# ShinYwings/SingleHDR-tf2

Measured on AMD Instinct MI355X. Metric: HDR images/sec (512x512) end-to-end inference, deq+lin+hal, higher is better.
Workload: dtype f32

## Files before the change

include/shdr.h:

```cpp
#ifndef SHDR_H_
#define SHDR_H_

#include <stdint.h>

#ifdef __cplusplus
extern "C" {
#endif

void shdr_config_reload(void);

#define SHDR_OK          0
#define SHDR_E_SHAPE    (-1)
#define SHDR_E_ALIGN    (-2)
#define SHDR_E_ARCH     (-3)
#define SHDR_E_LAUNCH   (-4)
#define SHDR_E_NULL     (-5)

#define SHDR_ACT_NONE   0
#define SHDR_ACT_RELU   1
#define SHDR_ACT_LRELU  2
#define SHDR_ACT_TANH   3

#define SHDR_ALGO_AUTO    0
#define SHDR_ALGO_MFMA    1
// ... 59 lines not shown
int64_t shdr_conv2d_workspace_bytes_f32(const shdr_conv2d_desc* d, int has_residual);
int shdr_conv2d_fwd_prepared_f32(const shdr_conv2d_desc* d, const float* x1, const float* x2, const float* prepared,
                                 const float* bias, const float* scale, const float* shift, const float* residual, float* y,
                                 float* y_pool, void* workspace, void* stream);
int shdr_conv2d_fwd_prepared_ranged_f32(const shdr_conv2d_desc* d, const float* x1, const float* x2, const float* prepared,
                                        const float* bias, const float* scale, const float* shift, const float* residual, float* y,
                                        float* y_pool, void* workspace, const float* x1_range, const float* x2_range, float* y_range,
                                        void* stream);
int shdr_conv2d_projected_ok_f32(const shdr_conv2d_desc* d);
int shdr_conv2d_fwd_prepared_projected_f32(const shdr_conv2d_desc* d, const float* x1, const float* x2, const float* prepared,
                                           const float* bias, const float* scale, const float* shift, const float* proj, float* y_proj,
                                           float* y, float* y_pool, void* workspace, const float* x1_range, const float* x2_range,
                                           float* y_range, void* stream);

int shdr_conv2d_up2_lowres_ok_f32(const shdr_conv2d_desc* d);
int64_t shdr_conv2d_up2_lowres_filter_elems_f32(const shdr_conv2d_desc* d);
int shdr_conv2d_up2_lowres_prepare_filter_f32(const shdr_conv2d_desc* d, const float* w, float* prepared, void* stream);
int64_t shdr_conv2d_up2_lowres_workspace_bytes_f32(const shdr_conv2d_desc* d);
int shdr_conv2d_fwd_up2_lowres_f32(const shdr_conv2d_desc* d, const float* x, const float* prepared, const float* bias,
                                   const float* scale, const float* shift, float* y, void* workspace, const float* x_range,
                                   float* y_range, void* stream);

int shdr_conv2d_up2_fused_ok_f32(const shdr_conv2d_desc* d);
int64_t shdr_conv2d_up2_fused_filter_elems_f32(const shdr_conv2d_desc* d);
int shdr_conv2d_up2_fused_prepare_filter_f32(const shdr_conv2d_desc* d, const float* w, float* prepared, void* stream);
int shdr_conv2d_fwd_up2_fused_f32(const shdr_conv2d_desc* d, const float* x, const float* prepared, const float* bias,
                                  const float* scale, const float* shift, const float* proj, float* y_proj, float* y,
                                  const float* x_range, float* y_range, void* stream);

int shdr_conv2d_wgrad_f32(const shdr_conv2d_desc* d, const float* x, int which, const float* dz,
                          float* dw, void* stream);
int shdr_filter_transform_f32(const float* w, float* wt, int KH, int KW, int Cin, int Cout,
                              int c_begin, int c_count, float scale, void* stream);
int64_t shdr_conv2d_dgrad_workspace_bytes_f32(const shdr_conv2d_desc* d, int which);
int shdr_conv2d_dgrad_f32(const shdr_conv2d_desc* d, int which, const float* dz, const float* w, float* dx, void* workspace,
                          void* stream);
int shdr_conv2d_dgrad_tracks_range_f32(const shdr_conv2d_desc* d, int which);
int shdr_conv2d_dgrad_ranged_f32(const shdr_conv2d_desc* d, int which, const float* dz, const float* w, float* dx, void* workspace,
                                 const float* dz_range, float* dx_range, void* stream);
enum { SHDR_OP_CONV2D_FWD = 0, SHDR_OP_CONV2D_DGRAD = 1, SHDR_OP_CONV2D_WGRAD_WINOGRAD = 2, SHDR_OP_BATCHNORM = 3,
       SHDR_OP_ACT_BWD_BIAS = 4  };
#define SHDR_BN_MAX_BLOCKS 1024
int64_t shdr_workspace_bytes(int op, const shdr_conv2d_desc* d, int arg);
int shdr_bias_grad_f32(const float* dz, float* db, int64_t npix, int C, void* stream);

int shdr_soft_hist_fwd_f32(const float* x, float* y, int64_t npix, int C, int B, void* stream);
// ... 358 lines not shown
```

singlehdr-tf2_amd/_lib.py:

```python
import ctypes
import os

_HERE = os.path.dirname(os.path.abspath(__file__))
LIB_PATH = os.environ.get("SHDR_LIB") or os.path.join(_HERE, "libshdr.so")

c_int = ctypes.c_int
c_i64 = ctypes.c_int64
c_f32 = ctypes.c_float
c_ptr = ctypes.c_void_p


class ConvDesc(ctypes.Structure):
    _fields_ = [("N", ctypes.c_int32), ("H", ctypes.c_int32), ("W", ctypes.c_int32),
                ("C1", ctypes.c_int32), ("C2", ctypes.c_int32),
                ("Cout", ctypes.c_int32), ("KH", ctypes.c_int32), ("KW", ctypes.c_int32),
                ("stride", ctypes.c_int32), ("pad_t", ctypes.c_int32), ("pad_l", ctypes.c_int32),
                ("Ho", ctypes.c_int32), ("Wo", ctypes.c_int32),
                ("x2_scale", ctypes.c_float),
                ("act1", ctypes.c_int32), ("act2", ctypes.c_int32),
                ("res_cstride", ctypes.c_int32), ("y_cstride", ctypes.c_int32),
                ("algo", ctypes.c_int32), ("cout_valid", ctypes.c_int32),
                ("w_batch_stride", ctypes.c_int64),
                ("y_pix_stride", ctypes.c_int32), ("y_off_h", ctypes.c_int32), ("y_off_w", ctypes.c_int32),
                ("y_H", ctypes.c_int32), ("y_W", ctypes.c_int32),
# ... 63 lines not shown
    "shdr_conv2d_fwd_x3n_ranged_f32": (c_int, [ctypes.POINTER(ConvDesc)] + [c_ptr] * 13),
    "shdr_act_bwd_bias_f32": (c_int, [c_ptr, c_ptr, c_ptr, c_ptr, c_ptr, c_i64, c_int, c_int, c_ptr]),
    "shdr_winograd_filter_packed_f32": (c_int, [c_ptr, c_ptr, c_int, c_int, c_ptr]),
    "shdr_conv2d_wgrad_winograd_f32": (c_int, [c_ptr] * 4 + [c_int] * 7 + [c_f32, c_ptr]),
    "shdr_crc32c": (ctypes.c_uint32, [c_ptr, ctypes.c_uint64, ctypes.c_uint32]),
    "shdr_same_pad": (c_int, [c_int, c_int, c_int, ctypes.POINTER(c_int), ctypes.POINTER(c_int)]),
    "shdr_conv2d_fwd_f32": (c_int, [ctypes.POINTER(ConvDesc)] + [c_ptr] * 9),
    "shdr_conv2d_fwd_yrange_f32": (c_int, [ctypes.POINTER(ConvDesc)] + [c_ptr] * 10),
    "shdr_conv2d_plan_f32": (c_int, [ctypes.POINTER(ConvDesc), c_int]),
    "shdr_conv2d_prepared_filter_elems_f32": (c_i64, [ctypes.POINTER(ConvDesc), c_int]),
    "shdr_conv2d_filter_is_plain_f32": (c_int, [ctypes.POINTER(ConvDesc), c_int]),
    "shdr_conv2d_prepare_filter_f32": (c_int, [ctypes.POINTER(ConvDesc), c_int, c_ptr, c_ptr, c_ptr]),
    "shdr_conv2d_workspace_bytes_f32": (c_i64, [ctypes.POINTER(ConvDesc), c_int]),
    "shdr_conv2d_fwd_prepared_f32": (c_int, [ctypes.POINTER(ConvDesc)] + [c_ptr] * 11),
    "shdr_conv2d_fwd_prepared_ranged_f32": (c_int, [ctypes.POINTER(ConvDesc)] + [c_ptr] * 14),
    "shdr_conv2d_projected_ok_f32": (c_int, [ctypes.POINTER(ConvDesc)]),
    "shdr_conv2d_fwd_prepared_projected_f32": (c_int, [ctypes.POINTER(ConvDesc)] + [c_ptr] * 15),
    "shdr_conv2d_up2_lowres_ok_f32": (c_int, [ctypes.POINTER(ConvDesc)]),
    "shdr_conv2d_up2_lowres_filter_elems_f32": (c_i64, [ctypes.POINTER(ConvDesc)]),
    "shdr_conv2d_up2_lowres_prepare_filter_f32": (c_int, [ctypes.POINTER(ConvDesc), c_ptr, c_ptr, c_ptr]),
    "shdr_conv2d_up2_lowres_workspace_bytes_f32": (c_i64, [ctypes.POINTER(ConvDesc)]),
    "shdr_conv2d_fwd_up2_lowres_f32": (c_int, [ctypes.POINTER(ConvDesc)] + [c_ptr] * 10),
    "shdr_conv2d_up2_fused_ok_f32": (c_int, [ctypes.POINTER(ConvDesc)]),
    "shdr_conv2d_up2_fused_filter_elems_f32": (c_i64, [ctypes.POINTER(ConvDesc)]),
    "shdr_conv2d_up2_fused_prepare_filter_f32": (c_int, [ctypes.POINTER(ConvDesc), c_ptr, c_ptr, c_ptr]),
    "shdr_conv2d_fwd_up2_fused_f32": (c_int, [ctypes.POINTER(ConvDesc)] + [c_ptr] * 11),
    "shdr_conv2d_fwd_x3_projected_f32": (c_int, [ctypes.POINTER(ConvDesc)] + [c_ptr] * 14),
    "shdr_conv2d_fwd_x3_residual_f32": (c_int, [ctypes.POINTER(ConvDesc)] + [c_ptr] * 12),
    "shdr_conv2d_dgrad_workspace_bytes_f32": (c_i64, [ctypes.POINTER(ConvDesc), c_int]),
    "shdr_conv2d_dgrad_f32": (c_int, [ctypes.POINTER(ConvDesc), c_int, c_ptr, c_ptr, c_ptr, c_ptr, c_ptr]),
    "shdr_conv2d_dgrad_tracks_range_f32": (c_int, [ctypes.POINTER(ConvDesc), c_int]),
    "shdr_conv2d_dgrad_ranged_f32": (c_int, [ctypes.POINTER(ConvDesc), c_int, c_ptr, c_ptr, c_ptr, c_ptr, c_ptr, c_ptr, c_ptr]),
    "shdr_workspace_bytes": (c_i64, [c_int, ctypes.POINTER(ConvDesc), c_int]),
    "shdr_soft_hist_bwd_f32": (c_int, [c_ptr, c_ptr, c_ptr, c_i64, c_int, c_int, c_ptr]),
    "shdr_conv2d_wgrad_f32": (c_int, [ctypes.POINTER(ConvDesc), c_ptr, c_int, c_ptr, c_ptr, c_ptr]),
    "shdr_filter_transform_f32": (c_int, [c_ptr, c_ptr, c_int, c_int, c_int, c_int, c_int, c_int, c_f32, c_ptr]),
    "shdr_bias_grad_f32": (c_int, [c_ptr, c_ptr, c_i64, c_int, c_ptr]),
    "shdr_soft_hist_fwd_f32": (c_int, [c_ptr, c_ptr, c_i64, c_int, c_int, c_ptr]),
    "shdr_lin_frontend_fwd_f32": (c_int, [c_ptr, c_ptr, c_int, c_int, c_int, c_int, c_ptr]),
    "shdr_avgpool2_fwd_f32": (c_int, [c_ptr, c_ptr, c_int, c_int, c_int, c_int, c_ptr]),
    "shdr_maxpool2_fwd_f32": (c_int, [c_ptr, c_ptr, c_int, c_int, c_int, c_int, c_ptr]),
    "shdr_maxpool3s2_fwd_f32": (c_int, [c_ptr, c_ptr, c_int, c_int, c_int, c_int, c_ptr]),
    "shdr_resize2x_fwd_f32": (c_int, [c_ptr, c_ptr, c_int, c_int, c_int, c_int, c_ptr]),
    "shdr_gap_fwd_f32": (c_int, [c_ptr, c_ptr, c_int, c_int, c_int, c_ptr]),
    "shdr_invcrf_decode_fwd_f32": (c_int, [c_ptr] * 5 + [c_int, c_int, c_int, c_ptr]),
    "shdr_increase_fwd_f32": (c_int, [c_ptr, c_ptr, c_int, c_int, c_ptr]),
# ... 116 lines not shown
```

singlehdr-tf2_amd/_ops.py:

```python
import collections
import ctypes
import math

import numpy as np
import torch

try:
    from . import _lib
except ImportError:
    import _lib

AUTOGRAD = None


def _needs_grad(*tensors):
    return AUTOGRAD is not None and torch.is_grad_enabled() and any(
        isinstance(t, torch.Tensor) and t.requires_grad for t in tensors)


WINOGRAD = True


ACT_NONE, ACT_RELU, ACT_LRELU, ACT_TANH = 0, 1, 2, 3
ALGO_AUTO, ALGO_MFMA, ALGO_DIRECT, ALGO_MFMA_REG = 0, 1, 2, 3
# ... 165 lines not shown
            raise NotImplementedError("conv2d: the native-fp16 path takes no pad / out / w_batch_stride / algo")
        if _needs_grad(x, x2, w, bias, scale, shift, residual):
            if fused:
                raise NotImplementedError("conv2d: the native-fp16 path takes bias + act1 only on a gradient tape (training-mode layers)")
            return AUTOGRAD.conv2d_h(x, w, bias, stride, x2, x2_scale, act1, cout_valid)
        return conv2d_h(x, pack_filter_h(w, x.shape[3], 0 if x2 is None else x2.shape[3], x2_scale), bias, tuple(w.shape[:2]),
                        w.shape[3], stride=stride, x2=x2, act1=act1, cout_valid=cout_valid, scale=scale, shift=shift,
                        residual=residual, act2=act2)
    if algo == ALGO_AUTO:
        algo = _AUTO_ALGO[PRECISION]
    fused = scale is not None or shift is not None or residual is not None or act2 != ACT_NONE
    if _needs_grad(x, x2, w, bias, scale, shift, residual):
        if pad is not None or out_hw is not None or out is not None or w_batch_stride:
            raise NotImplementedError("conv2d: pad / out_hw / out / w_batch_stride are raw-kernel options (input-gradient and "
                                      "Winograd plumbing) and cannot be recorded on a gradient tape")
        y = AUTOGRAD.conv2d(x, w, bias, stride=stride, x2=x2, x2_scale=x2_scale, act1=act1, algo=algo, cout_valid=cout_valid)
        if not fused:
            return y
        return AUTOGRAD.affine_act(y, scale, shift, residual, act2)
    return _conv2d_raw(x, w, bias, stride, x2, x2_scale, act1, scale, shift, residual, act2, algo, out, cout_valid, pad, out_hw,
                       w_batch_stride, None)


def conv2d_up2(x, w, bias=None, act1=ACT_NONE, scale=None, shift=None, act2=ACT_NONE, proj=None, lowres=False):
    if lowres and proj is not None and not _is_h(x) and _AUTO_ALGO[PRECISION] == ALGO_AUTO and WINOGRAD and not EXACT_FP32 \
            and not _needs_grad(x, w, bias, scale, shift):
        yj = _conv2d_up2_fused(x, w, bias, act1, scale, shift, act2, proj)
        if yj is not None:
            return yj
    if lowres and proj is None and not _is_h(x) and _AUTO_ALGO[PRECISION] == ALGO_AUTO and WINOGRAD and not EXACT_FP32 \
            and not _needs_grad(x, w, bias, scale, shift):
        y = _conv2d_up2_lowres(x, w, bias, act1, scale, shift, act2)
        if y is not None:
            return y
    algo = _AUTO_ALGO[PRECISION]
    if _is_h(x) or algo != ALGO_AUTO or not WINOGRAD or _needs_grad(x, w, bias, scale, shift):
        if proj is not None:
            return None
        return conv2d(resize2x(x), w, bias, act1=act1, scale=scale, shift=shift, act2=act2)
    return _conv2d_raw(x, w, bias, 1, None, 1.0, act1, scale, shift, None, act2, algo, None, None, None, None, 0, None,
                       prologue=PROLOGUE_BILINEAR2X, proj=proj)


def _up2_layer(form, x, w, bias, act1, scale, shift, act2):
    lib = _lib.load()
    x, w_var = _d(x), w
    w = _d(w)
    if x.dim() != 4 or w.dim() != 4 or tuple(w.shape[:2]) != (3, 3) or w.shape[2] != x.shape[3]:
        return None
    n, h, wd, c1 = x.shape
    cout = w.shape[3]
    d = _lib.ConvDesc()
    d.N, d.H, d.W, d.C1, d.C2 = n, 2 * h, 2 * wd, c1, 0
    d.Cout, d.KH, d.KW, d.stride = cout, 3, 3, 1
    d.cout_valid, d.y_cstride = cout, cout
    d.pad_t, d.pad_l, d.Ho, d.Wo = 1, 1, 2 * h, 2 * wd
    d.x2_scale = 1.0
    d.act1, d.act2 = act1, act2
    d.algo = ALGO_AUTO
    d.prologue = PROLOGUE_BILINEAR2X
    if not int(getattr(lib, "shdr_conv2d_up2_%s_ok_f32" % form)(ctypes.byref(d))):
        return None
    _chk(x, "x")
    _chk(w, "w")
# ... 13 lines not shown
    return d, x, prepared


def _conv2d_up2_lowres(x, w, bias, act1, scale, shift, act2):
    layer = _up2_layer("lowres", x, w, bias, act1, scale, shift, act2)
    if layer is None:
        return None
    lib = _lib.load()
    x_in = x
    d, x, prepared = layer
    xr = _range_of(x_in)
    if xr is None:
        RANGE_MISSES[(tuple(x.shape), None, tuple(_d(w).shape))] += 1
    ws = torch.empty(int(lib.shdr_conv2d_up2_lowres_workspace_bytes_f32(ctypes.byref(d))), device=x.device, dtype=torch.uint8)
    out = torch.empty((d.N, d.H, d.W, d.Cout), device=x.device, dtype=torch.float32)
    yr = _new_slot(x.device)
    rc = lib.shdr_conv2d_fwd_up2_lowres_f32(ctypes.byref(d), _ptr(x), _ptr(prepared), _ptr(_d(bias)), _ptr(_d(scale)), _ptr(_d(shift)),
                                            _ptr(out), _ptr(ws), _ptr(xr), _ptr(yr), _stream())
    _lib.check(rc, "shdr_conv2d_fwd_up2_lowres_f32")
    return _set_range(out, yr)


def _conv2d_up2_fused(x, w, bias, act1, scale, shift, act2, proj=None, want_y=None):
    layer = _up2_layer("fused", x, w, bias, act1, scale, shift, act2)
    if layer is None:
        return None
    lib = _lib.load()
    x_in = x
    d, x, prepared = layer
    if proj is not None:
        proj = _chk(_d(proj), "proj")
        if tuple(proj.shape) != (3, d.Cout):
            raise ValueError("conv2d_up2: proj must be [3, %d]" % d.Cout)
    if want_y is None:
        want_y = proj is None
    xr = _range_of(x_in)
    if xr is None:
        RANGE_MISSES[(tuple(x.shape), None, tuple(_d(w).shape))] += 1
        xr = _new_slot(x.device)
        _lib.check(lib.shdr_absmax_f32(_ptr(x), x.numel(), _ptr(xr), _stream()), "shdr_absmax_f32")
    out = torch.empty((d.N, d.H, d.W, d.Cout), device=x.device, dtype=torch.float32) if want_y else None
    yj = torch.empty((d.N, d.H, d.W, 3), device=x.device, dtype=torch.float32) if proj is not None else None
    yr = _new_slot(x.device) if want_y else None
    rc = lib.shdr_conv2d_fwd_up2_fused_f32(ctypes.byref(d), _ptr(x), _ptr(prepared), _ptr(_d(bias)), _ptr(_d(scale)), _ptr(_d(shift)),
                                           _ptr(proj), _ptr(yj), _ptr(out), _ptr(xr), _ptr(yr), _stream())
    _lib.check(rc, "shdr_conv2d_fwd_up2_fused_f32")
# ... 1843 lines not shown
```

singlehdr-tf2_amd/csrc/up2_fused.hip:

```cpp
#include <hip/hip_fp16.h>
#include <stdlib.h>

#include <type_traits>

#include "shdr_internal.h"

namespace {

using f32x4 = __attribute__((ext_vector_type(4))) float;
using f16x8 = __attribute__((ext_vector_type(8))) _Float16;

inline hipStream_t S(void* s) { return reinterpret_cast<hipStream_t>(s); }

constexpr int UF_HEADER_FLOATS = 16;
constexpr int UF_IMG_HALVES = 64 * 32, UF_UNIT_HALVES = 2 * UF_IMG_HALVES;
constexpr int UF_R = 8;
constexpr int UF_COLS = 14;
constexpr int UF_MAX_CIN = 128;
constexpr int UF_STRIDE = UF_MAX_CIN + 8;
constexpr int UF_THREADS = 256;

struct UpFusedArgs {
  const float* x;
  const _Float16* wp;
  const float* hdr;
  const float* bias;
  const float* scale;
  const float* shift;
  const float* proj;
  float* y;
  float* yproj;
  const unsigned* xr;
  unsigned* yr;
  int N, h, w, C1, nty, ntx, act1, act2;
};

__device__ __forceinline__ void uf_range_scale(const unsigned* r, float& xs, float& ixs) {
  xs = 1.0f;
  ixs = 1.0f;
  const unsigned b = r ? *r : 0u;
  if (b != 0u && b < 0x7f800000u) {
    int ex;
    frexpf(__uint_as_float(b), &ex);
    int T = 11 - ex;
    T = T < -126 ? -126 : (T > 126 ? 126 : T);
    xs = ldexpf(1.0f, T);
    ixs = ldexpf(1.0f, -T);
  }
}
__device__ __forceinline__ void uf_split4(const f32x4 v, float xs, unsigned (&h)[2], unsigned (&l)[2]) {
  const float k2048 = 2048.0f;
#pragma unroll
  for (int p = 0; p < 2; ++p) {
    float t0, t1;
    asm("v_fma_mixlo_f16 %0, %1, %2, 0" : "=v"(h[p]) : "v"(v[2 * p]), "s"(xs));
    asm("v_fma_mixhi_f16 %0, %1, %2, 0" : "+v"(h[p]) : "v"(v[2 * p + 1]), "s"(xs));
    asm("v_fma_mix_f32 %0, %1, %2, -%3 op_sel_hi:[0,0,1]" : "=v"(t0) : "v"(v[2 * p]), "s"(xs), "v"(h[p]));
// ... 19 lines not shown
  f32x4 r;
#pragma unroll
  for (int e = 0; e < 4; ++e) r[e] = __builtin_fmaf(a[e], s[e], c[e]);
  return r;
}
__device__ __forceinline__ f32x4 from_left(f32x4 a) {
  f32x4 r;
#pragma unroll
  for (int e = 0; e < 4; ++e) r[e] = __int_as_float(__builtin_amdgcn_update_dpp(0, __float_as_int(a[e]), 0x111, 0xf, 0xf, true));
  return r;
}
__device__ __forceinline__ f32x4 from_right(f32x4 a) {
  f32x4 r;
#pragma unroll
  for (int e = 0; e < 4; ++e) r[e] = __int_as_float(__builtin_amdgcn_update_dpp(0, __float_as_int(a[e]), 0x101, 0xf, 0xf, true));
  return r;
}

__device__ __forceinline__ int uf_xcd_remap(int bid, int nwg) {
  const int q = nwg >> 3, r = nwg & 7, xcd = bid & 7, idx = bid >> 3;
  return (xcd < r ? xcd * (q + 1) : r * (q + 1) + (xcd - r) * q) + idx;
}

template <int R>
__global__ __launch_bounds__(UF_THREADS, 2) void up2_fused_kernel(const UpFusedArgs a) {
  constexpr int NPIX = 16 * R, IMG = NPIX * UF_STRIDE;
  constexpr int RO = R - 2;
  extern __shared__ __attribute__((aligned(16))) _Float16 fsm[];

  const int tid = threadIdx.x, lane = tid & 63;
  const int cw = __builtin_amdgcn_readfirstlane(tid >> 6);
  int L = uf_xcd_remap(blockIdx.x, gridDim.x);
  const int tx_ = L % a.ntx; L /= a.ntx;
  const int ty_ = L % a.nty;
  const int n = L / a.nty;
  const int m_start = ty_ * RO, j_start = tx_ * UF_COLS;
  const int nch = a.C1 >> 5;

  float xs, ixs;
  {
    const int f4n = a.C1 >> 2, total = NPIX * f4n;
    const float* xb = a.x + (size_t)n * a.h * a.w * a.C1;
    uf_range_scale(a.xr, xs, ixs);
#pragma unroll 1
    for (int id0 = tid; id0 < total; id0 += 4 * UF_THREADS) {
      f32x4 v[4];
      int dst[4];
#pragma unroll
      for (int k = 0; k < 4; ++k) {
        const int id = id0 + k * UF_THREADS;
        dst[k] = -1;
        if (id < total) {
          const int pp = id / f4n, f = id - pp * f4n;
          const int row = min(max(m_start - 1 + (pp >> 4), 0), a.h - 1), col = min(max(j_start - 1 + (pp & 15), 0), a.w - 1);
          v[k] = *reinterpret_cast<const f32x4*>(xb + ((size_t)row * a.w + col) * a.C1 + 4 * f);
          dst[k] = pp * UF_STRIDE + 4 * f;
        }
      }
#pragma unroll
      for (int k = 0; k < 4; ++k) {
        if (dst[k] >= 0) {
          unsigned h[2], l[2];
          uf_split4(v[k], xs, h, l);
          *reinterpret_cast<uint2*>(fsm + dst[k]) = make_uint2(h[0], h[1]);
          *reinterpret_cast<uint2*>(fsm + IMG + dst[k]) = make_uint2(l[0], l[1]);
        }
      }
    }
  }
  __syncthreads();

  const int p = lane & 15, fg = lane >> 4;
  const int j0 = j_start - 1 + p;
  const bool lane_ok = p >= 1 && p <= UF_COLS && j0 < a.w;
  const float wl0 = j0 >= 1 ? 0.75f : 0.0f, wl1 = j0 >= 1 ? 0.25f : 0.0f;
  const float wr0 = j0 + 1 < a.w ? 0.25f : 0.0f, wr1 = j0 + 1 < a.w ? 0.75f : 0.0f;
  const float inv_s = a.hdr[1] * ixs;
  const _Float16* wlane = a.wp + (16 * cw + p) * 32 + 8 * fg;
  const _Float16* xlane = fsm + p * UF_STRIDE + 8 * fg;

  f32x4 out[RO][2][2];

  auto pass = [&](auto tyc) __attribute__((always_inline)) {
    constexpr int TY = decltype(tyc)::value;
    f32x4 z[3][R];
#pragma unroll
    for (int t = 0; t < 3; ++t)
#pragma unroll
      for (int q = 0; q < R; ++q) z[t][q] = (f32x4){0.f, 0.f, 0.f, 0.f};
    const _Float16* wt = wlane + (size_t)(3 * TY) * nch * UF_UNIT_HALVES;
#pragma unroll 1
    for (int c = 0; c < nch; ++c) {
      f16x8 wh[3], wl[3], ws[3];
#pragma unroll
      for (int t = 0; t < 3; ++t) {
        const _Float16* g = wt + ((size_t)t * nch + c) * UF_UNIT_HALVES;
        wh[t] = *reinterpret_cast<const f16x8*>(g);
        wl[t] = *reinterpret_cast<const f16x8*>(g + UF_IMG_HALVES);
      }
#pragma unroll
      for (int t = 0; t < 3; ++t) ws[t] = wh[t] * (_Float16)(1.0f / 2048.0f);
      const _Float16* xc = xlane + 32 * c;
#pragma unroll
      for (int q = 0; q < R; ++q) {
        const f16x8 ph = *reinterpret_cast<const f16x8*>(xc + q * 16 * UF_STRIDE);
        const f16x8 pl = *reinterpret_cast<const f16x8*>(xc + IMG + q * 16 * UF_STRIDE);
#pragma unroll
        for (int t = 0; t < 3; ++t) z[t][q] = __builtin_amdgcn_mfma_f32_16x16x32_f16(wh[t], ph, z[t][q], 0, 0, 0);
#pragma unroll
        for (int t = 0; t < 3; ++t) z[t][q] = __builtin_amdgcn_mfma_f32_16x16x32_f16(ws[t], pl, z[t][q], 0, 0, 0);
#pragma unroll
        for (int t = 0; t < 3; ++t) z[t][q] = __builtin_amdgcn_mfma_f32_16x16x32_f16(wl[t], ph, z[t][q], 0, 0, 0);
      }
    }
#pragma unroll
    for (int q = 0; q < R; ++q) {
      asm volatile("" : "+v"(z[0][q]), "+v"(z[1][q]), "+v"(z[2][q]));
      f32x4 zz[3];
#pragma unroll
// ... 31 lines not shown
        } else if (TY == 1) {
          if (q >= 2) out[q - 2][1][s] = fma4(H[s], 0.25f, out[q - 2][1][s]);
          if (q + 1 <= RO) out[q][0][s] = fma4(H[s], 0.25f, out[q][0][s]);
          if (q >= 1 && q <= RO) {
            out[q - 1][0][s] = fma4(H[s], 0.75f, out[q - 1][0][s]);
            out[q - 1][1][s] = fma4(H[s], 0.75f, out[q - 1][1][s]);
          }
        } else {
          if (q >= 2) {
            out[q - 2][0][s] = fma4(H[s], 0.25f, out[q - 2][0][s]);
            out[q - 2][1][s] = fma4(H[s], mq < a.h ? 0.75f : 0.0f, out[q - 2][1][s]);
          }
          if (q >= 1 && q <= RO) {
            out[q - 1][0][s] = fma4(H[s], 0.75f, out[q - 1][0][s]);
            out[q - 1][1][s] = fma4(H[s], mq + 1 < a.h ? 0.25f : 0.0f, out[q - 1][1][s]);
          }
        }
      }
      if (q >= 1 && q <= RO) asm volatile("" : "+v"(out[q - 1][0][0]), "+v"(out[q - 1][0][1]), "+v"(out[q - 1][1][0]), "+v"(out[q - 1][1][1]));
      if (q + 1 <= RO) asm volatile("" : "+v"(out[q][0][0]), "+v"(out[q][0][1]), "+v"(out[q][1][0]), "+v"(out[q][1][1]));
      if (q >= 2) asm volatile("" : "+v"(out[q - 2][0][0]), "+v"(out[q - 2][0][1]), "+v"(out[q - 2][1][0]), "+v"(out[q - 2][1][1]));
    }
  };
  pass(std::integral_constant<int, 0>{});
  pass(std::integral_constant<int, 1>{});
  pass(std::integral_constant<int, 2>{});

  const int c = 16 * cw + 4 * fg;
  auto ld = [](const float* q) __attribute__((always_inline)) { return *reinterpret_cast<const f32x4*>(q); };
  const f32x4 bias_r = a.bias ? ld(a.bias + c) : (f32x4){0.f, 0.f, 0.f, 0.f};
  const f32x4 scale_r = a.scale ? ld(a.scale + c) : (f32x4){1.f, 1.f, 1.f, 1.f};
  const f32x4 shift_r = a.scale ? ld(a.shift + c) : (f32x4){0.f, 0.f, 0.f, 0.f};
  f32x4 pq[3];
#pragma unroll
  for (int j = 0; j < 3; ++j) pq[j] = a.proj ? ld(a.proj + j * 64 + c) : (f32x4){0.f, 0.f, 0.f, 0.f};
  if (a.proj) __syncthreads();
  float* part = reinterpret_cast<float*>(fsm);
  float ym = 0.0f;
#pragma unroll
  for (int qo = 0; qo < RO; ++qo) {
    const int m0 = m_start + qo;
    const bool row_ok = m0 < a.h;
#pragma unroll
    for (int r = 0; r < 2; ++r)
#pragma unroll
      for (int s = 0; s < 2; ++s) {
        f32x4 v = out[qo][r][s];
        v += bias_r;
        shdr::act_apply4<0>(v, a.act1);
        if (a.scale) v = fma4v(v, scale_r, shift_r);
        shdr::act_apply4<0>(v, a.act2);
        if (a.y && row_ok && lane_ok) {
          *reinterpret_cast<f32x4*>(a.y + (((size_t)n * 2 * a.h + 2 * m0 + r) * 2 * a.w + 2 * j0 + s) * 64 + c) = v;
          ym = fmaxf(fmaxf(fmaxf(fmaxf(ym, fabsf(v[0])), fabsf(v[1])), fabsf(v[2])), fabsf(v[3]));
        }
        if (a.proj) {
#pragma unroll
          for (int j = 0; j < 3; ++j) {
            float t = v[0] * pq[j][0] + v[1] * pq[j][1] + v[2] * pq[j][2] + v[3] * pq[j][3];
            t += __shfl_xor(t, 16, 64);
            t += __shfl_xor(t, 32, 64);
            if (fg == 0) part[(cw * RO * 64 + (qo * 2 + r) * 32 + 2 * p + s) * 3 + j] = t;
          }
        }
      }
  }
  if (a.proj) {
    __syncthreads();
    for (int slot = tid; slot < RO * 64; slot += UF_THREADS) {
      const int s = slot & 1, pp = (slot >> 1) & 15, r = (slot >> 5) & 1, qo = slot >> 6;
      const int m0 = m_start + qo, jj = j_start - 1 + pp;
      if (m0 < a.h && pp >= 1 && pp <= UF_COLS && jj < a.w) {
        float* o = a.yproj + (((size_t)n * 2 * a.h + 2 * m0 + r) * 2 * a.w + 2 * jj + s) * 3;
#pragma unroll
        for (int j = 0; j < 3; ++j)
          o[j] = ((part[slot * 3 + j] + part[(RO * 64 + slot) * 3 + j]) + part[(2 * RO * 64 + slot) * 3 + j]) + part[(3 * RO * 64 + slot) * 3 + j];
      }
    }
  }
  if (a.y && a.yr) shdr::range_out_block256(a.yr, ym);
}

constexpr int uf_lds_bytes(int R) { return 2 * 16 * R * UF_STRIDE * 2; }

bool uf_shape_ok(const shdr_conv2d_desc* d) {
  return d && d->N > 0 && d->H > 0 && d->W > 0 && d->H % 2 == 0 && d->W % 2 == 0 && d->KH == 3 && d->KW == 3 && d->stride == 1 && d->pad_t == 1 &&
         d->pad_l == 1 && d->Ho == d->H && d->Wo == d->W && d->C2 == 0 && d->C1 % 32 == 0 && d->C1 >= 64 && d->C1 <= UF_MAX_CIN && d->Cout == 64;
}

}

extern "C" int shdr_conv2d_up2_fused_ok_f32(const shdr_conv2d_desc* d) {
  if (!uf_shape_ok(d) || SHDR_ENV("SHDR_NO_UP2_FUSED") != nullptr || SHDR_ENV("SHDR_NO_UP2_LOWRES") != nullptr || SHDR_ENV("SHDR_NO_WINOGRAD") != nullptr ||
      SHDR_ENV("SHDR_NO_X3") != nullptr)
    return 0;
  if (d->algo != SHDR_ALGO_AUTO || d->prologue != SHDR_PROLOGUE_BILINEAR2X) return 0;
  if ((d->cout_valid != 0 && d->cout_valid != d->Cout) || d->w_batch_stride != 0 || d->y_pix_stride > 1 || (d->y_cstride != 0 && d->y_cstride != d->Cout)) return 0;
  if (d->act1 == SHDR_ACT_TANH || d->act2 == SHDR_ACT_TANH) return 0;
  const long nblk = (long)d->N * ((d->H / 2 + UF_R - 3) / (UF_R - 2)) * ((d->W / 2 + UF_COLS - 1) / UF_COLS);
  return nblk <= 0x7fffffffL ? 1 : 0;
}

extern "C" int64_t shdr_conv2d_up2_fused_filter_elems_f32(const shdr_conv2d_desc* d) {
  return uf_shape_ok(d) ? shdr_conv2d_up2_lowres_filter_elems_f32(d) : -1;
}
extern "C" int shdr_conv2d_up2_fused_prepare_filter_f32(const shdr_conv2d_desc* d, const float* w, float* prepared, void* stream) {
  SHDR_REQUIRE(uf_shape_ok(d), SHDR_E_SHAPE, "up2_fused_prepare_filter: need a 3x3 layer with one source, Cin 64 / 96 / 128, Cout 64, even H and W");
  return shdr_conv2d_up2_lowres_prepare_filter_f32(d, w, prepared, stream);
}

extern "C" int shdr_conv2d_fwd_up2_fused_f32(const shdr_conv2d_desc* d, const float* x, const float* prepared, const float* bias, const float* scale,
                                             const float* shift, const float* proj, float* y_proj, float* y, const float* x_range, float* y_range,
                                             void* stream) {
  SHDR_REQUIRE(d && x && prepared && x_range, SHDR_E_NULL, "conv2d_up2_fused: null desc / x / prepared filter / x_range");
  SHDR_REQUIRE(y || y_proj, SHDR_E_NULL, "conv2d_up2_fused: neither y nor y_proj");
  SHDR_REQUIRE((proj == nullptr) == (y_proj == nullptr), SHDR_E_NULL, "conv2d_up2_fused: proj and y_proj come together");
  SHDR_REQUIRE(shdr_conv2d_up2_fused_ok_f32(d), SHDR_E_SHAPE, "conv2d_up2_fused: layer not taken (shdr_conv2d_up2_fused_ok_f32)");
  SHDR_REQUIRE((scale == nullptr) == (shift == nullptr), SHDR_E_NULL, "conv2d_up2_fused: scale and shift come together");
  SHDR_REQUIRE(shdr::aligned16(x) && shdr::aligned16(prepared) && (!y || shdr::aligned16(y)) && (!bias || shdr::aligned16(bias)) &&
                   (!scale || (shdr::aligned16(scale) && shdr::aligned16(shift))) && (!proj || shdr::aligned16(proj)),
               SHDR_E_ALIGN, "conv2d_up2_fused: tensors must be 16-byte aligned");
  UpFusedArgs a{};
  a.x = x; a.hdr = prepared; a.wp = reinterpret_cast<const _Float16*>(prepared + UF_HEADER_FLOATS);
  a.bias = bias; a.scale = scale; a.shift = shift; a.proj = proj; a.y = y; a.yproj = y_proj;
  a.xr = reinterpret_cast<const unsigned*>(x_range); a.yr = reinterpret_cast<unsigned*>(y_range);
  a.N = d->N; a.h = d->H / 2; a.w = d->W / 2; a.C1 = d->C1; a.act1 = d->act1; a.act2 = d->act2;
  a.nty = (a.h + UF_R - 3) / (UF_R - 2);
  a.ntx = (a.w + UF_COLS - 1) / UF_COLS;
  constexpr int lds = uf_lds_bytes(UF_R);
  static bool attr_done[shdr::kMaxDevices] = {};
  const int dev_slot = shdr::device_slot();
  if (!attr_done[dev_slot]) {
    hipError_t e = hipFuncSetAttribute(reinterpret_cast<const void*>(&up2_fused_kernel<UF_R>), hipFuncAttributeMaxDynamicSharedMemorySize, lds);
    if (e != hipSuccess) return shdr::fail(SHDR_E_ARCH, "hipFuncSetAttribute: %s", hipGetErrorString(e));
    attr_done[dev_slot] = true;
  }
  const long nblk = (long)a.N * a.nty * a.ntx;
  hipLaunchKernelGGL((up2_fused_kernel<UF_R>), dim3((unsigned)nblk), dim3(UF_THREADS), lds, S(stream), a);
  return shdr::check_launch("up2_fused_kernel");
}
```

singlehdr-tf2_amd/dequantization_net.py:

```python
import torch

try:
    from . import _ops as K
    from ._layers import Layer, Conv2D
except ImportError:
    import _ops as K
    from _layers import Layer, Conv2D


class down(Layer):

    def __init__(self, inChannels, outChannels, kernel_size=(3, 3), device=None):
        super().__init__()
        self.conv1 = Conv2D(inChannels, outChannels, kernel_size, device=device)
        self.conv2 = Conv2D(outChannels, outChannels, kernel_size, device=device)

    def call(self, x):
        x = K.avgpool2(x)
        x = self.conv1(x, act1=K.ACT_LRELU)
        return self.conv2(x, act1=K.ACT_LRELU)

    def call_pooled(self, xp):
        x = self.conv1(xp, act1=K.ACT_LRELU)
        return self.conv2.call_avgpool2(x, act1=K.ACT_LRELU)


class up(Layer):

    def __init__(self, inChannels, skipChannels, outChannels, kernel_size=3, device=None):
        super().__init__()
        self.conv1 = Conv2D(inChannels, outChannels, kernel_size, device=device)
        self.conv2 = Conv2D(outChannels + skipChannels, outChannels, kernel_size, device=device)

    def call(self, x, skpCn):
        x = self.conv1.call_up2(x, act1=K.ACT_LRELU)
        return self.conv2(x, x2=skpCn, act1=K.ACT_LRELU)


class _unet(Layer):
    def __init__(self, in_channels, bottleneck, device=None):
        super().__init__()
        self.conv1 = Conv2D(in_channels, 16, (7, 7), device=device)
        self.conv2 = Conv2D(16, 16, (7, 7), device=device)
        self.d2 = down(16, 32, (5, 5), device=device)
        self.d3 = down(32, 64, (3, 3), device=device)
        self.d4 = down(64, 128, (3, 3), device=device)
        self.enc = down(128, bottleneck, (3, 3), device=device)
        self.u4 = up(bottleneck, 128, 128, device=device)
        self.u3 = up(128, 64, 64, device=device)
        self.u2 = up(64, 32, 32, device=device)
        self.u1 = up(32, 16, 16, device=device)
        self.out = Conv2D(16, 3, (3, 3), device=device)

    def _trunk(self, input_images):
        cin = input_images.shape[-1]
        if cin == 3 and K.native_fp16():
            x = self.conv1.call_padded(K.pack3([input_images], 8, K.HALF), cin_pad=8, act1=K.ACT_LRELU)
        elif cin == 3:
# ... 26 lines not shown
```

Baseline: 924.2.

## Extend fused up2 conv kernel to narrow Cout 32/16 layers in dequantization UNet

```diff
diff --git a/include/shdr.h b/include/shdr.h
--- a/include/shdr.h
+++ b/include/shdr.h
@@ -105,6 +105,7 @@
                                    float* y_range, void* stream);
 
 int shdr_conv2d_up2_fused_ok_f32(const shdr_conv2d_desc* d);
+int shdr_conv2d_up2_narrow_enabled(void);
 int64_t shdr_conv2d_up2_fused_filter_elems_f32(const shdr_conv2d_desc* d);
 int shdr_conv2d_up2_fused_prepare_filter_f32(const shdr_conv2d_desc* d, const float* w, float* prepared, void* stream);
 int shdr_conv2d_fwd_up2_fused_f32(const shdr_conv2d_desc* d, const float* x, const float* prepared, const float* bias,
diff --git a/singlehdr-tf2_amd/_lib.py b/singlehdr-tf2_amd/_lib.py
--- a/singlehdr-tf2_amd/_lib.py
+++ b/singlehdr-tf2_amd/_lib.py
@@ -109,6 +109,7 @@
     "shdr_conv2d_up2_lowres_workspace_bytes_f32": (c_i64, [ctypes.POINTER(ConvDesc)]),
     "shdr_conv2d_fwd_up2_lowres_f32": (c_int, [ctypes.POINTER(ConvDesc)] + [c_ptr] * 10),
     "shdr_conv2d_up2_fused_ok_f32": (c_int, [ctypes.POINTER(ConvDesc)]),
+    "shdr_conv2d_up2_narrow_enabled": (c_int, []),
     "shdr_conv2d_up2_fused_filter_elems_f32": (c_i64, [ctypes.POINTER(ConvDesc)]),
     "shdr_conv2d_up2_fused_prepare_filter_f32": (c_int, [ctypes.POINTER(ConvDesc), c_ptr, c_ptr, c_ptr]),
     "shdr_conv2d_fwd_up2_fused_f32": (c_int, [ctypes.POINTER(ConvDesc)] + [c_ptr] * 11),
diff --git a/singlehdr-tf2_amd/_ops.py b/singlehdr-tf2_amd/_ops.py
--- a/singlehdr-tf2_amd/_ops.py
+++ b/singlehdr-tf2_amd/_ops.py
@@ -211,7 +211,7 @@
                        w_batch_stride, None)
 
 
-def conv2d_up2(x, w, bias=None, act1=ACT_NONE, scale=None, shift=None, act2=ACT_NONE, proj=None, lowres=False):
+def conv2d_up2(x, w, bias=None, act1=ACT_NONE, scale=None, shift=None, act2=ACT_NONE, proj=None, lowres=False, one_launch=False):
     if lowres and proj is not None and not _is_h(x) and _AUTO_ALGO[PRECISION] == ALGO_AUTO and WINOGRAD and not EXACT_FP32 \
             and not _needs_grad(x, w, bias, scale, shift):
         yj = _conv2d_up2_fused(x, w, bias, act1, scale, shift, act2, proj)
@@ -219,6 +219,10 @@
             return yj
     if lowres and proj is None and not _is_h(x) and _AUTO_ALGO[PRECISION] == ALGO_AUTO and WINOGRAD and not EXACT_FP32 \
             and not _needs_grad(x, w, bias, scale, shift):
+        if one_launch and up2_narrow_enabled():
+            y = _conv2d_up2_fused(x, w, bias, act1, scale, shift, act2)
+            if y is not None:
+                return y
         y = _conv2d_up2_lowres(x, w, bias, act1, scale, shift, act2)
         if y is not None:
             return y
@@ -229,6 +233,10 @@
         return conv2d(resize2x(x), w, bias, act1=act1, scale=scale, shift=shift, act2=act2)
     return _conv2d_raw(x, w, bias, 1, None, 1.0, act1, scale, shift, None, act2, algo, None, None, None, None, 0, None,
                        prologue=PROLOGUE_BILINEAR2X, proj=proj)
+
+
+def up2_narrow_enabled():
+    return bool(_lib.load().shdr_conv2d_up2_narrow_enabled())
 
 
 def _up2_layer(form, x, w, bias, act1, scale, shift, act2):
@@ -288,6 +296,8 @@
 
 
 def _conv2d_up2_fused(x, w, bias, act1, scale, shift, act2, proj=None, want_y=None):
+    if proj is not None and _d(w).shape[-1] != 64:
+        return None
     layer = _up2_layer("fused", x, w, bias, act1, scale, shift, act2)
     if layer is None:
         return None
diff --git a/singlehdr-tf2_amd/csrc/up2_fused.hip b/singlehdr-tf2_amd/csrc/up2_fused.hip
--- a/singlehdr-tf2_amd/csrc/up2_fused.hip
+++ b/singlehdr-tf2_amd/csrc/up2_fused.hip
@@ -17,8 +17,8 @@
 constexpr int UF_R = 8;
 constexpr int UF_COLS = 14;
 constexpr int UF_MAX_CIN = 128;
-constexpr int UF_STRIDE = UF_MAX_CIN + 8;
 constexpr int UF_THREADS = 256;
+constexpr int uf_stride(int CMAX) { return CMAX == 32 ? 32 : CMAX + 8; }
 
 struct UpFusedArgs {
   const float* x;
@@ -33,6 +33,7 @@
   const unsigned* xr;
   unsigned* yr;
   int N, h, w, C1, nty, ntx, act1, act2;
+  int npatch;
 };
 
 __device__ __forceinline__ void uf_range_scale(const unsigned* r, float& xs, float& ixs) {
@@ -98,15 +99,24 @@
   return (xcd < r ? xcd * (q + 1) : r * (q + 1) + (xcd - r) * q) + idx;
 }
 
-template <int R>
+template <int R, int CW, int CMAX>
 __global__ __launch_bounds__(UF_THREADS, 2) void up2_fused_kernel(const UpFusedArgs a) {
+  constexpr int UF_STRIDE = uf_stride(CMAX);
+  constexpr int COUT = 16 * CW, PPB = 4 / CW, GT = 64 * CW;
   constexpr int NPIX = 16 * R, IMG = NPIX * UF_STRIDE;
   constexpr int RO = R - 2;
-  extern __shared__ __attribute__((aligned(16))) _Float16 fsm[];
-
-  const int tid = threadIdx.x, lane = tid & 63;
-  const int cw = __builtin_amdgcn_readfirstlane(tid >> 6);
-  int L = uf_xcd_remap(blockIdx.x, gridDim.x);
+  extern __shared__ __attribute__((aligned(16))) _Float16 fsm_all[];
+
+  const int lane = threadIdx.x & 63;
+  const int wave = __builtin_amdgcn_readfirstlane(threadIdx.x >> 6);
+  const int ps = PPB == 1 ? 0 : wave / CW;
+  const int cw = PPB == 1 ? wave : wave % CW;
+  const int tid = PPB == 1 ? threadIdx.x : threadIdx.x & (GT - 1);
+  _Float16* const fsm = fsm_all + ps * (2 * IMG);
+  const float* const projp = CW == 4 ? a.proj : nullptr;
+  int L = uf_xcd_remap(blockIdx.x, gridDim.x) * PPB + ps;
+  const bool patch_ok = PPB == 1 || L < a.npatch;
+  if (!patch_ok) L = 0;
   const int tx_ = L % a.ntx; L /= a.ntx;
   const int ty_ = L % a.nty;
   const int n = L / a.nty;
@@ -119,12 +129,12 @@
     const float* xb = a.x + (size_t)n * a.h * a.w * a.C1;
     uf_range_scale(a.xr, xs, ixs);
 #pragma unroll 1
-    for (int id0 = tid; id0 < total; id0 += 4 * UF_THREADS) {
+    for (int id0 = patch_ok ? tid : total; id0 < total; id0 += 4 * GT) {
       f32x4 v[4];
       int dst[4];
 #pragma unroll
       for (int k = 0; k < 4; ++k) {
-        const int id = id0 + k * UF_THREADS;
+        const int id = id0 + k * GT;
         dst[k] = -1;
         if (id < total) {
           const int pp = id / f4n, f = id - pp * f4n;
@@ -152,7 +162,7 @@
   const float wl0 = j0 >= 1 ? 0.75f : 0.0f, wl1 = j0 >= 1 ? 0.25f : 0.0f;
   const float wr0 = j0 + 1 < a.w ? 0.25f : 0.0f, wr1 = j0 + 1 < a.w ? 0.75f : 0.0f;
   const float inv_s = a.hdr[1] * ixs;
-  const _Float16* wlane = a.wp + (16 * cw + p) * 32 + 8 * fg;
+  const _Float16* wlane = a.wp + p * 32 + 8 * fg;
   const _Float16* xlane = fsm + p * UF_STRIDE + 8 * fg;
 
   f32x4 out[RO][2][2];
@@ -164,13 +174,18 @@
     for (int t = 0; t < 3; ++t)
 #pragma unroll
       for (int q = 0; q < R; ++q) z[t][q] = (f32x4){0.f, 0.f, 0.f, 0.f};
-    const _Float16* wt = wlane + (size_t)(3 * TY) * nch * UF_UNIT_HALVES;
+    size_t wo[3];
+#pragma unroll
+    for (int t = 0; t < 3; ++t) {
+      const int col = (3 * TY + t) * COUT + 16 * cw;
+      wo[t] = (size_t)(col >> 6) * nch * UF_UNIT_HALVES + (col & 63) * 32;
+    }
 #pragma unroll 1
     for (int c = 0; c < nch; ++c) {
       f16x8 wh[3], wl[3], ws[3];
 #pragma unroll
       for (int t = 0; t < 3; ++t) {
-        const _Float16* g = wt + ((size_t)t * nch + c) * UF_UNIT_HALVES;
+        const _Float16* g = wlane + wo[t] + (size_t)c * UF_UNIT_HALVES;
         wh[t] = *reinterpret_cast<const f16x8*>(g);
         wl[t] = *reinterpret_cast<const f16x8*>(g + UF_IMG_HALVES);
       }
@@ -248,9 +263,11 @@
       if (q >= 2) asm volatile("" : "+v"(out[q - 2][0][0]), "+v"(out[q - 2][0][1]), "+v"(out[q - 2][1][0]), "+v"(out[q - 2][1][1]));
     }
   };
-  pass(std::integral_constant<int, 0>{});
-  pass(std::integral_constant<int, 1>{});
-  pass(std::integral_constant<int, 2>{});
+  if (patch_ok) {
+    pass(std::integral_constant<int, 0>{});
+    pass(std::integral_constant<int, 1>{});
+    pass(std::integral_constant<int, 2>{});
+  }
 
   const int c = 16 * cw + 4 * fg;
   auto ld = [](const float* q) __attribute__((always_inline)) { return *reinterpret_cast<const f32x4*>(q); };
@@ -259,14 +276,14 @@
   const f32x4 shift_r = a.scale ? ld(a.shift + c) : (f32x4){0.f, 0.f, 0.f, 0.f};
   f32x4 pq[3];
 #pragma unroll
-  for (int j = 0; j < 3; ++j) pq[j] = a.proj ? ld(a.proj + j * 64 + c) : (f32x4){0.f, 0.f, 0.f, 0.f};
-  if (a.proj) __syncthreads();
+  for (int j = 0; j < 3; ++j) pq[j] = projp ? ld(projp + j * 64 + c) : (f32x4){0.f, 0.f, 0.f, 0.f};
+  if (projp) __syncthreads();
   float* part = reinterpret_cast<float*>(fsm);
   float ym = 0.0f;
 #pragma unroll
   for (int qo = 0; qo < RO; ++qo) {
     const int m0 = m_start + qo;
-    const bool row_ok = m0 < a.h;
+    const bool row_ok = patch_ok && m0 < a.h;
 #pragma unroll
     for (int r = 0; r < 2; ++r)
 #pragma unroll
@@ -277,10 +294,10 @@
         if (a.scale) v = fma4v(v, scale_r, shift_r);
         shdr::act_apply4<0>(v, a.act2);
         if (a.y && row_ok && lane_ok) {
-          *reinterpret_cast<f32x4*>(a.y + (((size_t)n * 2 * a.h + 2 * m0 + r) * 2 * a.w + 2 * j0 + s) * 64 + c) = v;
+          *reinterpret_cast<f32x4*>(a.y + (((size_t)n * 2 * a.h + 2 * m0 + r) * 2 * a.w + 2 * j0 + s) * COUT + c) = v;
           ym = fmaxf(fmaxf(fmaxf(fmaxf(ym, fabsf(v[0])), fabsf(v[1])), fabsf(v[2])), fabsf(v[3]));
         }
-        if (a.proj) {
+        if (projp) {
 #pragma unroll
           for (int j = 0; j < 3; ++j) {
             float t = v[0] * pq[j][0] + v[1] * pq[j][1] + v[2] * pq[j][2] + v[3] * pq[j][3];
@@ -291,7 +308,7 @@
         }
       }
   }
-  if (a.proj) {
+  if (projp) {
     __syncthreads();
     for (int slot = tid; slot < RO * 64; slot += UF_THREADS) {
       const int s = slot & 1, pp = (slot >> 1) & 15, r = (slot >> 5) & 1, qo = slot >> 6;
@@ -307,32 +324,87 @@
   if (a.y && a.yr) shdr::range_out_block256(a.yr, ym);
 }
 
-constexpr int uf_lds_bytes(int R) { return 2 * 16 * R * UF_STRIDE * 2; }
-
-bool uf_shape_ok(const shdr_conv2d_desc* d) {
+constexpr int uf_lds_bytes(int R, int CW, int CMAX) { return (4 / CW) * 2 * 16 * R * uf_stride(CMAX) * 2; }
+
+bool uf_geometry_ok(const shdr_conv2d_desc* d) {
   return d && d->N > 0 && d->H > 0 && d->W > 0 && d->H % 2 == 0 && d->W % 2 == 0 && d->KH == 3 && d->KW == 3 && d->stride == 1 && d->pad_t == 1 &&
-         d->pad_l == 1 && d->Ho == d->H && d->Wo == d->W && d->C2 == 0 && d->C1 % 32 == 0 && d->C1 >= 64 && d->C1 <= UF_MAX_CIN && d->Cout == 64;
-}
-
-}
+         d->pad_l == 1 && d->Ho == d->H && d->Wo == d->W && d->C2 == 0 && d->C1 % 32 == 0 && d->C1 <= UF_MAX_CIN;
+}
+bool uf_shape_ok(const shdr_conv2d_desc* d) { return uf_geometry_ok(d) && d->C1 >= 64 && d->Cout == 64; }
+bool uf_narrow_shape_ok(const shdr_conv2d_desc* d) {
+  return uf_geometry_ok(d) && d->C1 >= 32 && (d->Cout == 32 || (d->Cout == 16 && d->C1 <= 64));
+}
+inline int uf_narrow_columns(int Cout) { return (9 * Cout + 63) / 64 * 64; }
+bool uf_narrow_gemm_desc(const shdr_conv2d_desc* d, shdr_conv2d_desc* g) {
+  if (!uf_narrow_shape_ok(d)) return false;
+  *g = shdr_conv2d_desc{};
+  g->N = d->N; g->H = d->H / 2; g->W = d->W / 2; g->C1 = d->C1; g->C2 = 0;
+  g->Cout = uf_narrow_columns(d->Cout);
+  g->KH = 1; g->KW = 1; g->stride = 1; g->pad_t = 0; g->pad_l = 0; g->Ho = g->H; g->Wo = g->W;
+  g->x2_scale = 1.0f; g->act1 = SHDR_ACT_NONE; g->act2 = SHDR_ACT_NONE; g->algo = SHDR_ALGO_AUTO; g->cout_valid = g->Cout; g->y_cstride = g->Cout;
+  return true;
+}
+__global__ __launch_bounds__(256) void up2_fused_filter_kernel(const float* __restrict__ w, float* __restrict__ st, int Cin, int Cout, int Cp) {
+  const long total = (long)Cin * Cp;
+  for (long e = (long)blockIdx.x * 256 + threadIdx.x; e < total; e += (long)gridDim.x * 256) {
+    const int col = (int)(e % Cp), ci = (int)(e / Cp);
+    const int t = col / Cout, co = col - t * Cout;
+    st[e] = t < 9 ? w[((size_t)t * Cin + ci) * Cout + co] : 0.0f;
+  }
+}
+
+template <int CW, int CMAX>
+int uf_launch(const UpFusedArgs& a, hipStream_t st) {
+  constexpr int lds = uf_lds_bytes(UF_R, CW, CMAX), PPB = 4 / CW;
+  static_assert(lds <= 160 * 1024 - 64, "the patch images of a block must fit the CU's LDS");
+  static bool attr_done[shdr::kMaxDevices] = {};
+  const int dev_slot = shdr::device_slot();
+  if (!attr_done[dev_slot]) {
+    hipError_t e = hipFuncSetAttribute(reinterpret_cast<const void*>(&up2_fused_kernel<UF_R, CW, CMAX>), hipFuncAttributeMaxDynamicSharedMemorySize, lds);
+    if (e != hipSuccess) return shdr::fail(SHDR_E_ARCH, "hipFuncSetAttribute: %s", hipGetErrorString(e));
+    attr_done[dev_slot] = true;
+  }
+  const long nblk = ((long)a.npatch + PPB - 1) / PPB;
+  hipLaunchKernelGGL((up2_fused_kernel<UF_R, CW, CMAX>), dim3((unsigned)nblk), dim3(UF_THREADS), lds, st, a);
+  return shdr::check_launch("up2_fused_kernel");
+}
+
+}
+
+extern "C" int shdr_conv2d_up2_narrow_enabled(void) { return SHDR_ENV("SHDR_NO_UP2_NARROW") == nullptr ? 1 : 0; }
 
 extern "C" int shdr_conv2d_up2_fused_ok_f32(const shdr_conv2d_desc* d) {
-  if (!uf_shape_ok(d) || SHDR_ENV("SHDR_NO_UP2_FUSED") != nullptr || SHDR_ENV("SHDR_NO_UP2_LOWRES") != nullptr || SHDR_ENV("SHDR_NO_WINOGRAD") != nullptr ||
-      SHDR_ENV("SHDR_NO_X3") != nullptr)
+  const bool narrow = uf_narrow_shape_ok(d) && shdr_conv2d_up2_narrow_enabled();
+  if (!(uf_shape_ok(d) || narrow) || SHDR_ENV("SHDR_NO_UP2_FUSED") != nullptr || SHDR_ENV("SHDR_NO_UP2_LOWRES") != nullptr ||
+      SHDR_ENV("SHDR_NO_WINOGRAD") != nullptr || SHDR_ENV("SHDR_NO_X3") != nullptr)
     return 0;
   if (d->algo != SHDR_ALGO_AUTO || d->prologue != SHDR_PROLOGUE_BILINEAR2X) return 0;
   if ((d->cout_valid != 0 && d->cout_valid != d->Cout) || d->w_batch_stride != 0 || d->y_pix_stride > 1 || (d->y_cstride != 0 && d->y_cstride != d->Cout)) return 0;
   if (d->act1 == SHDR_ACT_TANH || d->act2 == SHDR_ACT_TANH) return 0;
   const long nblk = (long)d->N * ((d->H / 2 + UF_R - 3) / (UF_R - 2)) * ((d->W / 2 + UF_COLS - 1) / UF_COLS);
-  return nblk <= 0x7fffffffL ? 1 : 0;
+  return nblk <= 0x7fffffffL - (narrow ? 4 : 0) ? 1 : 0;
 }
 
 extern "C" int64_t shdr_conv2d_up2_fused_filter_elems_f32(const shdr_conv2d_desc* d) {
-  return uf_shape_ok(d) ? shdr_conv2d_up2_lowres_filter_elems_f32(d) : -1;
+  if (uf_shape_ok(d)) return shdr_conv2d_up2_lowres_filter_elems_f32(d);
+  shdr_conv2d_desc g;
+  if (!uf_narrow_gemm_desc(d, &g)) return -1;
+  const int64_t packed = shdr_conv2d_x3_filter_elems_f32(&g);
+  return packed < 0 ? -1 : packed + (int64_t)g.C1 * g.Cout;
 }
 extern "C" int shdr_conv2d_up2_fused_prepare_filter_f32(const shdr_conv2d_desc* d, const float* w, float* prepared, void* stream) {
-  SHDR_REQUIRE(uf_shape_ok(d), SHDR_E_SHAPE, "up2_fused_prepare_filter: need a 3x3 layer with one source, Cin 64 / 96 / 128, Cout 64, even H and W");
-  return shdr_conv2d_up2_lowres_prepare_filter_f32(d, w, prepared, stream);
+  if (uf_shape_ok(d)) return shdr_conv2d_up2_lowres_prepare_filter_f32(d, w, prepared, stream);
+  SHDR_REQUIRE(d && w && prepared, SHDR_E_NULL, "up2_fused_prepare_filter: null pointer");
+  shdr_conv2d_desc g;
+  SHDR_REQUIRE(uf_narrow_gemm_desc(d, &g), SHDR_E_SHAPE,
+               "up2_fused_prepare_filter: need a 3x3 layer with one source, even H and W, and Cin 64 / 96 / 128 -> 64, Cin 32 .. 128 -> 32 or Cin 32 / 64 -> 16");
+  const int64_t packed = shdr_conv2d_x3_filter_elems_f32(&g);
+  SHDR_REQUIRE(packed > 0, SHDR_E_SHAPE, "up2_fused_prepare_filter: the 1x1 form of this layer has no packed filter");
+  float* staged = prepared + packed;
+  const long total = (long)g.C1 * g.Cout;
+  hipLaunchKernelGGL(up2_fused_filter_kernel, dim3(shdr::stream_grid(total)), dim3(256), 0, S(stream), w, staged, g.C1, d->Cout, g.Cout);
+  if (int rc = shdr::check_launch("up2_fused_filter")) return rc;
+  return shdr_conv2d_x3_prepare_filter_f32(&g, staged, prepared, stream);
 }
 
 extern "C" int shdr_conv2d_fwd_up2_fused_f32(const shdr_conv2d_desc* d, const float* x, const float* prepared, const float* bias, const float* scale,
@@ -342,6 +414,7 @@
   SHDR_REQUIRE(y || y_proj, SHDR_E_NULL, "conv2d_up2_fused: neither y nor y_proj");
   SHDR_REQUIRE((proj == nullptr) == (y_proj == nullptr), SHDR_E_NULL, "conv2d_up2_fused: proj and y_proj come together");
   SHDR_REQUIRE(shdr_conv2d_up2_fused_ok_f32(d), SHDR_E_SHAPE, "conv2d_up2_fused: layer not taken (shdr_conv2d_up2_fused_ok_f32)");
+  SHDR_REQUIRE(!proj || d->Cout == 64, SHDR_E_SHAPE, "conv2d_up2_fused: the projected output is the 64-cout form's");
   SHDR_REQUIRE((scale == nullptr) == (shift == nullptr), SHDR_E_NULL, "conv2d_up2_fused: scale and shift come together");
   SHDR_REQUIRE(shdr::aligned16(x) && shdr::aligned16(prepared) && (!y || shdr::aligned16(y)) && (!bias || shdr::aligned16(bias)) &&
                    (!scale || (shdr::aligned16(scale) && shdr::aligned16(shift))) && (!proj || shdr::aligned16(proj)),
@@ -353,15 +426,9 @@
   a.N = d->N; a.h = d->H / 2; a.w = d->W / 2; a.C1 = d->C1; a.act1 = d->act1; a.act2 = d->act2;
   a.nty = (a.h + UF_R - 3) / (UF_R - 2);
   a.ntx = (a.w + UF_COLS - 1) / UF_COLS;
-  constexpr int lds = uf_lds_bytes(UF_R);
-  static bool attr_done[shdr::kMaxDevices] = {};
-  const int dev_slot = shdr::device_slot();
-  if (!attr_done[dev_slot]) {
-    hipError_t e = hipFuncSetAttribute(reinterpret_cast<const void*>(&up2_fused_kernel<UF_R>), hipFuncAttributeMaxDynamicSharedMemorySize, lds);
-    if (e != hipSuccess) return shdr::fail(SHDR_E_ARCH, "hipFuncSetAttribute: %s", hipGetErrorString(e));
-    attr_done[dev_slot] = true;
-  }
-  const long nblk = (long)a.N * a.nty * a.ntx;
-  hipLaunchKernelGGL((up2_fused_kernel<UF_R>), dim3((unsigned)nblk), dim3(UF_THREADS), lds, S(stream), a);
-  return shdr::check_launch("up2_fused_kernel");
-}
+  a.npatch = (int)((long)a.N * a.nty * a.ntx);
+  hipStream_t st = S(stream);
+  if (d->Cout == 64) return uf_launch<4, 128>(a, st);
+  if (d->Cout == 32) return d->C1 <= 64 ? uf_launch<2, 64>(a, st) : uf_launch<2, 128>(a, st);
+  return d->C1 <= 32 ? uf_launch<1, 32>(a, st) : uf_launch<1, 64>(a, st);
+}
diff --git a/singlehdr-tf2_amd/dequantization_net.py b/singlehdr-tf2_amd/dequantization_net.py
--- a/singlehdr-tf2_amd/dequantization_net.py
+++ b/singlehdr-tf2_amd/dequantization_net.py
@@ -2,10 +2,10 @@
 
 try:
     from . import _ops as K
-    from ._layers import Layer, Conv2D
+    from ._layers import Layer, Conv2D, taping
 except ImportError:
     import _ops as K
-    from _layers import Layer, Conv2D
+    from _layers import Layer, Conv2D, taping
 
 
 class down(Layer):
@@ -33,7 +33,11 @@
         self.conv2 = Conv2D(outChannels + skipChannels, outChannels, kernel_size, device=device)
 
     def call(self, x, skpCn):
-        x = self.conv1.call_up2(x, act1=K.ACT_LRELU)
+        if x.dtype == torch.float32 and K.WINOGRAD and not K.EXACT_FP32 and K.up2_narrow_enabled() \
+                and not taping(x, self.conv1.kernel, self.conv1.bias):
+            x = self.conv1.call_up2(x, act1=K.ACT_LRELU, lowres=True, one_launch=True)
+        else:
+            x = self.conv1.call_up2(x, act1=K.ACT_LRELU)
         return self.conv2(x, x2=skpCn, act1=K.ACT_LRELU)
 
 
```

New measurement: 947.2, median of 6. +2.5%, better.
